# nomadkaraoke/python-audio-separator

Hardware: AMD Instinct MI355X
Metric: audio-sec separated / wall-sec (RTF), UVR-MDX-NET 44.1kHz stereo, 1/2/4/8 GPU (higher is better)
Workload: dtype f32 (I/O and accumulators; matrix products on the 16-bit pipe from block-scaled two-part fp16 operands, 22-bit products -- see arithmetic; fp32-exact setting timed in arithmetic_ab)

## Files before the change

python-audio-separator_amd/csrc/asx.hip:

```cpp
#include <hip/hip_runtime.h>

#include <algorithm>
#include <atomic>
#include <cmath>
#include <cstdarg>
#include <cstdio>
#include <cstdlib>
#include <cstring>
#include <functional>
#include <map>
#include <string>
#include <mutex>
#include <vector>

#include "../../include/asx.h"
#include "knobs.h"

static void grant_lds(const void *kernel, int bytes) {
  static std::mutex mu;
  static std::map<const void *, int> granted;
  std::lock_guard<std::mutex> lock(mu);
  int &g = granted[kernel];
  if (bytes > g) {
    (void)hipFuncSetAttribute(kernel, hipFuncAttributeMaxDynamicSharedMemorySize, bytes);
// ... 27 lines not shown
#include "engine_core.h"
#include "engine_mdx.h"

static int opt_nonneg(int32_t v) { return v < 0 ? 0 : (int)v; }
static int opt_onoff(int32_t v) { return v > 0 ? 1 : 0; }

static const struct EngineOption {
  const char *key;
  int asx_engine::*field;
  int EngineKnobs::*knob;
  int (*norm)(int32_t);
  const char *refusal = nullptr;
  int shipped = 0;
} kOptions[] = {
    {"winograd", &asx_engine::winograd, &EngineKnobs::winograd, opt_nonneg,
     "asx_set_option: winograd = %d names a superseded kernel generation that only an experimental build carries "
     "(python build.py --experimental); this library has 0 (direct kernel) and 3 (the default)", 3},
    {"winograd_stationary", &asx_engine::winos, &EngineKnobs::winos, opt_nonneg,
     "asx_set_option: the weight-stationary Winograd kernel (measured slower) is in experimental builds only (python build.py --experimental)"},
    {"winograd_bf16x6", &asx_engine::wino6, &EngineKnobs::wino6, opt_nonneg},
    {"gemm_bf16x6", &asx_engine::gemm_bf16x6, &EngineKnobs::gemm_bf16x6, opt_onoff},
    {"gemm_f16x3", &asx_engine::gemm_f16x3, &EngineKnobs::gemm_f16x3, opt_onoff},
    {"conv_direct_f16x3", &asx_engine::conv3h, &EngineKnobs::conv3h, opt_nonneg},
    {"conv_down_bf16x6", &asx_engine::down6, &EngineKnobs::down6, opt_onoff},
    {"conv_up_bf16x6", &asx_engine::up6, &EngineKnobs::up6, opt_onoff},
    {"gemm_pair_images", &asx_engine::pair_images, &EngineKnobs::pair_images, opt_onoff,
     "asx_set_option: gemm_pair_images = 1 needs an experimental build (python build.py --experimental): the pair-image reader measured no "
     "faster in the nets and is not in the default library"},
};

static const EngineOption *find_option(const char *fn, const char *key) {
  for (const EngineOption &o : kOptions)
    if (!strcmp(key, o.key)) return &o;
  set_err("%s: unknown option '%s'", fn, key);
  return nullptr;
}

extern "C" {

int asx_abi_version(void) { return ASX_ABI_VERSION; }
const char *asx_last_error(void) { return g_err; }

int asx_device_count(void) {
  int n = 0;
  if (hipGetDeviceCount(&n) != hipSuccess) return 0;
  return n;
// ... 111 lines not shown
    return rc;
  }
  *out = e;
  return ASX_OK;
}

static void v3_destroy(V3Net *n);
static void rof_destroy(RofNet *n);
static void ht_destroy(HtNet *n);
static void hd_destroy(HdNet *n);
static void hd_drop_clones(asx_engine *e);
static void vr_destroy(VrNet *n);
static void ens_destroy(EnsCtx *c);
static void free_conv(ConvLayer &L) {
  L.w.release();
  L.b.release();
  L.wu.release();
  L.wu2.release();
  L.wu3.release();
  L.wus.release();
  L.wu6.release();
  L.wu6h.release();
  L.w3h.release();
  L.wd6.release();
  L.wup6.release();
  L.gn_w.release();
  L.gn_b.release();
}
static void free_tdf(TdfLayer &L) {
  L.w.release();
  L.bias.release();
  L.scale.release();
  L.shift.release();
  L.gn_w.release();
  L.gn_b.release();
}
static void free_block(Block &b) {
  for (auto &c : b.tfc) free_conv(c);
  free_tdf(b.tdf0);
  free_tdf(b.tdf1);
}

void asx_engine_destroy(asx_engine *e) {
  w3_flush(e);
  if (!e) return;
  (void)hipSetDevice(e->device);
// ... 1859 lines not shown
  CHK(vr_plan(*e->vr, n_samples, &T, &n_out));
  DevBuf dw, dp, ds;
  BufGuard g{{&dw, &dp, &ds}};
  CHK(to_dev(dw, wave_host, (size_t)2 * n_samples));
  if (primary_host) CHK(dp.ensure((size_t)2 * n_out * 4));
  if (secondary_host) CHK(ds.ensure((size_t)2 * n_out * 4));
  CHK(vr_separate_dev(e, dw.f(), n_samples, params, primary_host ? dp.f() : nullptr, secondary_host ? ds.f() : nullptr, nullptr));
  if (primary_host) CHK(to_host(primary_host, dp, (size_t)2 * n_out));
  if (secondary_host) CHK(to_host(secondary_host, ds, (size_t)2 * n_out));
  return ASX_OK;
}

int asx_counter(const asx_engine *e, const char *name, int64_t *out) {
  REQUIRE(e && name && out, "asx_counter: null argument");
  const std::string nm(name);
  if (nm == "tdf3_launches") *out = (int64_t)g_tdf3_launches.load();
  else if (nm == "tdf3h_launches") *out = (int64_t)g_tdf3h_launches.load();
  else if (nm == "attn6_launches") *out = (int64_t)g_attn6_launches.load();
  else if (nm == "attn6h_launches") *out = (int64_t)g_attn6h_launches.load();
  else if (nm == "tdf3_gather_launches") *out = (int64_t)g_tdf3_gather_launches.load();
  else if (nm == "wino6_launches") *out = (int64_t)g_wino6_launches.load();
  else if (nm == "wino6h_launches") *out = (int64_t)g_wino6h_launches.load();
  else if (nm == "conv3h_launches") *out = (int64_t)g_conv3h_launches.load();
  else if (nm == "tdf3_pair_image_launches") *out = (int64_t)g_tdf3ps_launches.load();
  else if (nm == "down6_launches") *out = (int64_t)g_down6_launches.load();
  else if (nm == "up6_launches") *out = (int64_t)g_up6_launches.load();
  else if (nm == "hd_rounds") *out = (int64_t)g_hd_rounds.load();
  else {
    set_err("asx_counter: unknown counter '%s'", name);
    return ASX_ERR_INVALID;
  }
  return ASX_OK;
}

int asx_debug_trace(uint64_t *host, int64_t n_u64) {
  REQUIRE(host && n_u64 > 0 && n_u64 <= 4096 * 8, "asx_debug_trace: bad argument");
  HIPCHK(hipDeviceSynchronize());
  HIPCHK(hipMemcpyFromSymbol(host, HIP_SYMBOL(asx_dbg_trace), (size_t)n_u64 * 8));
  return ASX_OK;
}

int asx_debug_fetch(asx_engine *e, const char *name, float *host, int64_t numel) {
  REQUIRE(e && name && host && numel > 0, "asx_debug_fetch: bad argument");
  HIPCHK(hipSetDevice(e->device));
  const float *src = nullptr;
  const std::string nm(name);
// ... 194 lines not shown
```

python-audio-separator_amd/csrc/engine_core.h:

```cpp
#pragma once

static thread_local char g_err[512] = "";
static void set_err(const char *fmt, ...) {
  va_list ap;
  va_start(ap, fmt);
  vsnprintf(g_err, sizeof(g_err), fmt, ap);
  va_end(ap);
}
#define HIPCHK(x)                                                                       \
  do {                                                                                  \
    hipError_t e_ = (x);                                                                \
    if (e_ != hipSuccess) {                                                             \
      set_err("%s:%d %s -> %s", __FILE__, __LINE__, #x, hipGetErrorString(e_));         \
      return ASX_ERR_HIP;                                                               \
    }                                                                                   \
  } while (0)
#define CHK(x)                    \
  do {                            \
    int r_ = (x);                 \
    if (r_ != ASX_OK) return r_;  \
  } while (0)
#define REQUIRE(cond, ...)        \
  do {                            \
    if (!(cond)) {                \
// ... 55 lines not shown
  CHK(run(din.f(), dout.f()));
  return to_host(out_host, dout, n_out);
}

enum ConvKind { CK_3X3 = 0, CK_DOWN = 1, CK_1X1 = 2, CK_UP = 3 };

struct ConvLayer {
  int kind = CK_3X3;
  int cin = 0, cout = 0;
  int nrep = 0, kc = 0, cg = 0, nci = 0;
  int relu = 1;
  DevBuf w, b;
  DevBuf wu;
  DevBuf wu2;
  DevBuf wu3;
  int wu_cg = 0, wu_nci = 0, wu3_nci = 0;
  DevBuf wus;
  int wus_ks = 0;
  DevBuf gn_w, gn_b;
  DevBuf wu6;
  int wu6_nci = 0;
  DevBuf wu6h;
  DevBuf w3h;
  DevBuf wd6;
  int wd6_cg = 0, wd6_nst = 0, wd6_nrep = 3;
  DevBuf wup6;
  int wup6_cg = 0, wup6_nst = 0;
};

struct TdfLayer {
  int n = 0, k = 0, c = 0;
  bool has_bias = false;
  DevBuf w, bias, scale, shift;
  DevBuf gn_w, gn_b;
};

struct Block {
  std::vector<ConvLayer> tfc;
  TdfLayer tdf0, tdf1;
  int c = 0, t = 0, f = 0;
};

struct ProfRec {
  int cls;
  int nprod;
  hipEvent_t a, b;
// ... 49 lines not shown
  bool net_begun = false, net_ready = false;
  asx_net_config net{};
  std::map<std::string, std::vector<float>> host_tensors;
  ConvLayer first, final_;
  std::vector<Block> enc, dec;
  Block mid;
  std::vector<ConvLayer> ds, us;
  int ws_batch = 0;
  DevBuf spec_in, spec_out, R[3], H, HE, frames, chunk_out, d_starts, d_nact, d_peak, d_demixed;
  DevBuf pool_wave, pool_nsong, pool_songs, pool_div, pool_peak;
  DevBuf gn_part;
  DevBuf d_div;
  DivKey div_key;
  DevBuf sinc_tab;
  hipEvent_t div_ev = nullptr;
  hipStream_t div_stream = nullptr;
  std::vector<DevBuf> skip;
  int winograd = 3;
  int winos = 0;
  int gemm_bf16x6 = 1;
  int gemm_f16x3 = 1;
  int wino6 = 144;
  int conv3h = 144;
  int down6 = 1;
  int up6 = 1;
  int pair_images = 0;
  std::vector<W3Entry> w3;
  std::mutex w3_mu;
  bool prof = false;
  int prof_nprod = 0;
  std::vector<ProfRec> recs;
};

static int pick_batch(const asx_engine *e) { return e->cfg.max_batch > 0 ? e->cfg.max_batch : 64; }

static int even_batches(int nk, int maxB) {
  const int nbatch = (nk + maxB - 1) / maxB;
  return (nk + nbatch - 1) / nbatch;
}

template <class F>
static int timed(asx_engine *e, int cls, double flops, double bytes, hipStream_t s, F &&launch) {
  if (!e->prof) {
    launch();
    HIPCHK(hipGetLastError());
    return ASX_OK;
// ... 68 lines not shown
```

python-audio-separator_amd/csrc/engine_mdx.h:

```cpp
#pragma once

template <class CFG>
static void launch_conv_t(const ConvArgs &a, int nblk, hipStream_t s) {
  grant_lds(&conv_mfma_kernel<CFG>, CFG::LDS_BYTES);
  hipLaunchKernelGGL(conv_mfma_kernel<CFG>, dim3(nblk), dim3(256), CFG::LDS_BYTES, s, a);
}

static int conv_tile_h(int kind) { return kind == CK_UP ? 4 : 8; }

static int pick_nrep_conv(int cout) {
  const int ct = (cout + 15) / 16;
  int best = 1, best_pad = 1 << 30;
  for (int n = 3; n >= 1; --n) {
    const int pad = ((ct + n - 1) / n) * n - ct;
    if (pad < best_pad) {
      best_pad = pad;
      best = n;
    }
  }
  return best;
}
static int pick_nrep_up(int cout) {
  const int ct = (cout + 15) / 16;
  if (knobs().up_nrep == 4 && (4 * ct) % 4 == 0) return 4;
// ... 128 lines not shown
#endif
#ifdef ASX_EXPERIMENTAL_KERNELS
    if (L.wus_ks) {
      const size_t per = (size_t)8 * (6 * L.wus_ks / 4) * 64 * 4;
      std::vector<float> wus((size_t)L.wu_cg * per, 0.f);
      for (int co = 0; co < L.cout; ++co)
        for (int c = 0; c < L.cin; ++c) {
          const float *g = &w[((size_t)co * L.cin + c) * 9];
          double t[4][3];
          for (int a = 0; a < 4; ++a)
            for (int j = 0; j < 3; ++j) t[a][j] = G[a][0] * g[0 * 3 + j] + G[a][1] * g[1 * 3 + j] + G[a][2] * g[2 * 3 + j];
          float *dst = &wus[(size_t)(co / 48) * per];
          for (int a = 0; a < 4; ++a)
            for (int bb = 0; bb < 4; ++bb) {
              const float u = (float)(t[a][0] * G[bb][0] + t[a][1] * G[bb][1] + t[a][2] * G[bb][2]);
              dst[L.wus_ks == 12 ? winos_u_index<12>(a, bb, c, co % 48) : winos_u_index<24>(a, bb, c, co % 48)] = u;
            }
        }
      CHK(L.wus.ensure(wus.size() * 4));
      HIPCHK(hipMemcpy(L.wus.p, wus.data(), wus.size() * 4, hipMemcpyHostToDevice));
    }
#endif
  }
  if (L.kind == CK_DOWN) {
    std::vector<uint32_t> w6;
    L.wd6_nrep = (knobs().down6_wide && L.cout % 96 == 0) ? 6 : 3;
    if (L.wd6_nrep == 6) down6_pack<6>(w, L.cout, L.cin, w6, &L.wd6_cg, &L.wd6_nst);
    else down6_pack<3>(w, L.cout, L.cin, w6, &L.wd6_cg, &L.wd6_nst);
    CHK(L.wd6.ensure(w6.size() * 4));
    HIPCHK(hipMemcpy(L.wd6.p, w6.data(), w6.size() * 4, hipMemcpyHostToDevice));
  }
  if (L.kind == CK_UP) {
    std::vector<uint32_t> w6;
    if (L.nrep == 6) up6_pack<6>(w, L.cout, L.cin, w6, &L.wup6_cg, &L.wup6_nst);
    else if (L.nrep == 4) up6_pack<4>(w, L.cout, L.cin, w6, &L.wup6_cg, &L.wup6_nst);
    else up6_pack<2>(w, L.cout, L.cin, w6, &L.wup6_cg, &L.wup6_nst);
    CHK(L.wup6.ensure(w6.size() * 4));
    HIPCHK(hipMemcpy(L.wup6.p, w6.data(), w6.size() * 4, hipMemcpyHostToDevice));
  }
  const int nb = (L.kind == CK_UP) ? CT * 16 : std::max(L.cg * NW, ((L.cout + 47) / 48) * 48);
  std::vector<float> bp(nb, 0.f);
  for (int i = 0; i < L.cout; ++i) bp[i] = b ? b[i] : 0.f;
  CHK(L.w.ensure(wp.size() * 4));
  CHK(L.b.ensure(bp.size() * 4));
  HIPCHK(hipMemcpy(L.w.p, wp.data(), wp.size() * 4, hipMemcpyHostToDevice));
  HIPCHK(hipMemcpy(L.b.p, bp.data(), bp.size() * 4, hipMemcpyHostToDevice));
  return ASX_OK;
}

template <class CFG>
static void launch_conv_dma_t(const ConvArgs &a, int nblk, hipStream_t s) {
  grant_lds(&conv_dma_kernel<CFG>, CFG::LDS_BYTES);
  hipLaunchKernelGGL(conv_dma_kernel<CFG>, dim3(nblk), dim3(256), CFG::LDS_BYTES, s, a);
}

static std::atomic<long long> g_wino6_launches{0};
static std::atomic<long long> g_wino6h_launches{0};
static std::atomic<long long> g_conv3h_launches{0};
static std::atomic<long long> g_down6_launches{0};
static std::atomic<long long> g_up6_launches{0};

struct ConvView {
  int64_t x_bstride = 0;
  int64_t y_bstride = 0;
  const float *res = nullptr;
  int64_t aux_bstride = 0;
  int act = -1;
  float alpha = 1.f;
};

static int conv_launch(asx_engine *e, const ConvLayer &L, const float *x, const float *skip, float *y, int B, int T,
                       int F, hipStream_t s, const ConvView &v = ConvView()) {
  ConvArgs a{};
  a.x = x;
  a.wp = L.w.f();
  a.bias = L.b.f();
  a.skip = skip;
  a.res = v.res;
  a.zeros = e->d_zeros.f();
  a.y = y;
  a.B = B;
  a.Cin = L.cin;
  a.Cout = L.cout;
  a.T = T;
  a.F = F;
  a.act = v.act >= 0 ? v.act : (L.relu ? ACT_RELU : ACT_NONE);
  a.alpha = v.alpha;
  REQUIRE(a.act != ACT_ELU || L.kind == CK_1X1, "ELU epilogue: 1x1 convolutions only");
  a.CG = L.cg;
  a.NCI = L.nci;
  a.nt = knobs().nt & 1;
  int cls = ASX_PROF_CONV3X3;
// ... 12 lines not shown
    if (L.kind == CK_1X1) {
      cls = ASX_PROF_CONV1X1;
      taps = 1;
    } else if (L.kind == CK_UP) {
      cls = ASX_PROF_UP;
      taps = 4;
      out_plane = (int64_t)4 * T * F;
    }
  }
  a.x_bstride = v.x_bstride ? v.x_bstride : (int64_t)L.cin * T * F;
  a.y_bstride = v.y_bstride ? v.y_bstride : (int64_t)L.cout * out_plane;
  a.aux_bstride = v.aux_bstride ? v.aux_bstride : (int64_t)L.cout * out_plane;
  const int th = conv_tile_h(L.kind);
  a.tilesT = (a.To + th - 1) / th;
  a.tilesF = (a.Fo + 63) / 64;
  const int nblk = a.CG * a.tilesT * a.tilesF * B;
  if (nblk <= 0) return ASX_OK;
  const double outpix = (double)B * a.To * a.Fo;
  const double flops = 2.0 * taps * L.cin * L.cout * outpix;
  double bytes = 4.0 * ((double)B * L.cin * T * F + (double)L.cout * outpix * (L.kind == CK_UP ? 4 : 1));
  if (L.kind == CK_UP && skip) bytes += 4.0 * (double)L.cout * outpix * 4;
  if (v.res) bytes += 4.0 * (double)L.cout * outpix;
  int bad = 0;
  const bool dma = (F % 4 == 0) && ((reinterpret_cast<uintptr_t>(x) & 15) == 0) && (a.x_bstride % 4 == 0) && !knobs().no_dma;
  const ConvArgs &d = a;
#ifdef ASX_EXPERIMENTAL_KERNELS
  if (L.kind == CK_3X3 && e->winograd == 3 && e->winos == 1 && dma && L.wus.p != nullptr && a.Fo % 32 == 0 && v.res == nullptr &&
      (a.act == ACT_RELU || a.act == ACT_NONE) && (int64_t)L.cin * T * F < ((int64_t)1 << 30)) {
    ConvArgs wa = a;
    wa.wp = L.wus.f();
    wa.CG = L.wu_cg;
    wa.tilesF = a.Fo / 32;
    const int NS = (a.To + 1) / 2;
    const int base = wa.CG * wa.tilesF * B;
    int RB = std::max(1, std::min((NS + 7) / 8, (2048 + base - 1) / base));
    const int SPB = (NS + RB - 1) / RB;
    RB = (NS + SPB - 1) / SPB;
    wa.tilesT = RB;
    wa.NCI = SPB;
    const int nb = base * RB;
    auto gos = [&](auto kern, int lds) {
      grant_lds(kern, lds);
      return timed(e, cls, flops, bytes, s, [&]() { hipLaunchKernelGGL(kern, dim3(nb), dim3(512), lds, s, wa); });
    };
    const int abls = knobs().winos_abl;
    const bool k12 = L.wus_ks == 12;
    const bool ragged = (a.To & 1) || (L.cout % 48) != 0;
    if (abls && !ragged) {
      switch (abls) {
        case 1: return k12 ? gos(&conv_winos_kernel<12, 1>, WinoSCfg<12>::LDS_BYTES) : gos(&conv_winos_kernel<24, 1>, WinoSCfg<24>::LDS_BYTES);
        case 2: return k12 ? gos(&conv_winos_kernel<12, 2>, WinoSCfg<12>::LDS_BYTES) : gos(&conv_winos_kernel<24, 2>, WinoSCfg<24>::LDS_BYTES);
        case 4: return k12 ? gos(&conv_winos_kernel<12, 4>, WinoSCfg<12>::LDS_BYTES) : gos(&conv_winos_kernel<24, 4>, WinoSCfg<24>::LDS_BYTES);
        case 5: return k12 ? gos(&conv_winos_kernel<12, 5>, WinoSCfg<12>::LDS_BYTES) : gos(&conv_winos_kernel<24, 5>, WinoSCfg<24>::LDS_BYTES);
        case 13: return k12 ? gos(&conv_winos_kernel<12, 13>, WinoSCfg<12>::LDS_BYTES) : gos(&conv_winos_kernel<24, 13>, WinoSCfg<24>::LDS_BYTES);
        default: break;
      }
    }
    if (ragged) return k12 ? gos(&conv_winos_kernel<12, 0, true>, WinoSCfg<12>::LDS_BYTES) : gos(&conv_winos_kernel<24, 0, true>, WinoSCfg<24>::LDS_BYTES);
    return k12 ? gos(&conv_winos_kernel<12, 0, false>, WinoSCfg<12>::LDS_BYTES) : gos(&conv_winos_kernel<24, 0, false>, WinoSCfg<24>::LDS_BYTES);
  }
#endif
  if (L.kind == CK_3X3 && e->winograd == 3 && e->gemm_bf16x6 > 0 && e->gemm_f16x3 > 0 && e->conv3h > 0 && L.cin <= e->conv3h && L.w3h.p != nullptr && dma &&
      v.res == nullptr && (a.act == ACT_RELU || a.act == ACT_NONE) && F % 32 == 0 && (int64_t)Conv3hCfg::C * T * F < ((int64_t)1 << 29) &&
      a.y_bstride % 4 == 0 && (reinterpret_cast<uintptr_t>(y) & 15) == 0) {
    const int nb = L.cin / Conv3hCfg::C;
    const int tilesT = (T + 3) / 4, tilesF = F / 32;
    int bw = 32;
    double best = 1e30;
    for (int cand : {32, 16, 8}) {
      if ((tilesT * cand) % 32 != 0) continue;
      const int tps = tilesT * cand / 32;
      const int bands = (tilesF + cand - 1) / cand, items = B * bands;
      const double cost = (double)(bands * cand) / tilesF * (tps + 1.0) / tps * (double)((items + 7) / 8) / (items / 8.0);
      if (cost < best - 1e-9) {
        best = cost;
        bw = cand;
      }
    }
    if (best > 1e29) bw = 32;
    grant_lds(&conv3h_kernel<0, false>, Conv3hCfg::LDS_BYTES);
    grant_lds(&conv3h_kernel<0, true>, Conv3hCfg::LDS_BYTES);
    const int64_t plane = (int64_t)T * F;
    return timed(e, cls, flops, bytes, s, [&]() {
      e->prof_nprod = 3;
      for (int ob = 0; ob < nb; ++ob)
        for (int ib = 0; ib < nb; ++ib) {
          Conv3hArgs ca{};
          ca.x = x + (int64_t)ib * Conv3hCfg::C * plane;
          ca.y = y + (int64_t)ob * Conv3hCfg::C * plane;
          ca.prev = ib > 0 ? ca.y : nullptr;
          ca.wimg = reinterpret_cast<const u32x4 *>(reinterpret_cast<const uint32_t *>(L.w3h.p) + (size_t)(ob * nb + ib) * Conv3hCfg::IMG_U32);
          ca.bias = ib == 0 ? L.b.f() + ob * Conv3hCfg::C : nullptr;
          ca.B = B;
          ca.T = T;
          ca.F = F;
          ca.x_bstride = a.x_bstride;
          ca.y_bstride = a.y_bstride;
          ca.act = ib == nb - 1 ? a.act : ACT_NONE;
          ca.tilesT = tilesT;
          ca.tilesF = tilesF;
          ca.bw = bw;
          ca.tps = (tilesT * bw) % 32 == 0 ? tilesT * bw / 32 : tilesT;
          if (ib > 0) hipLaunchKernelGGL((conv3h_kernel<0, true>), dim3(256), dim3(512), Conv3hCfg::LDS_BYTES, s, ca);
          else hipLaunchKernelGGL((conv3h_kernel<0, false>), dim3(256), dim3(512), Conv3hCfg::LDS_BYTES, s, ca);
          g_conv3h_launches.fetch_add(1);
        }
    });
  }
  if (L.kind == CK_3X3 && e->winograd == 3 && e->gemm_bf16x6 > 0 && e->wino6 > 0 && L.cin >= e->wino6 && dma && L.wu6_nci > 0 &&
      (int64_t)T * F < ((int64_t)1 << 24)) {
    ConvArgs wa = a;
    const bool h3 = e->gemm_f16x3 > 0 && L.wu6h.p != nullptr;
    wa.wp = reinterpret_cast<const float *>(h3 ? L.wu6h.p : L.wu6.p);
    wa.CG = L.wu_cg;
    wa.NCI = L.wu6_nci;
    wa.tilesT = (a.To + Wino6Cfg::TH - 1) / Wino6Cfg::TH;
    wa.tilesF = (a.Fo + Wino6Cfg::TW - 1) / Wino6Cfg::TW;
    const int64_t S = (int64_t)wa.tilesT * wa.tilesF * B;
    const int64_t nb = ((S + 7) / 8) * 8 * wa.CG;
    if (nb < ((int64_t)1 << 31)) {
      grant_lds(&conv_wino6_kernel<0, 1>, Wino6Cfg::LDS_BYTES);
      grant_lds(&conv_wino6_kernel<0, 1, true>, Wino6Cfg::LDS_BYTES);
      g_wino6_launches.fetch_add(1);
      if (h3) g_wino6h_launches.fetch_add(1);
      return timed(e, cls, flops, bytes, s, [&]() {
        e->prof_nprod = h3 ? 3 : 6;
// ... 655 lines not shown
      else hipLaunchKernelGGL(f3::istft3p_kernel<0>, dim3(ng, 2, B), dim3(256), f3::ISTFT3P_LDS_BYTES, s, f);
    }
    else
      hipLaunchKernelGGL(f3::istft3_kernel, dim3(ng, 2, B), dim3(256), f3::ISTFT3_LDS_BYTES, s, f);
    if (ng > 1) hipLaunchKernelGGL(f3::seam3_kernel, dim3(5, ng - 1, B * 2), dim3(256), 0, s, f);
  });
}

static int gn_launch(asx_engine *e, const float *x, int B, int C, int64_t P, const DevBuf &gw, const DevBuf &gb, const float *res,
                     const float *mul, float *y, hipStream_t s) {
  if (B <= 0) return ASX_OK;
  REQUIRE(C % 2 == 0 && gw.p && gb.p && e->gn_part.bytes >= (size_t)B * C * 16, "GroupNorm(2, %d): channels / workspace", C);
  double2 *part = reinterpret_cast<double2 *>(e->gn_part.p);
  const double bytes = 4.0 * (double)B * C * (double)P;
  CHK(timed(e, ASX_PROF_MISC, 0.0, bytes, s,
            [&]() { hipLaunchKernelGGL(gn_partial_kernel, dim3((unsigned)C, (unsigned)B), dim3(256), 0, s, x, C, P, part); }));
  const int nx = (int)std::max<int64_t>(1, std::min<int64_t>(32, (P / 4 + 1023) / 1024));
  return timed(e, ASX_PROF_MISC, 0.0, bytes * (2 + (res ? 1 : 0) + (mul ? 1 : 0)), s, [&]() {
    hipLaunchKernelGGL(gn_apply_kernel, dim3((unsigned)nx, (unsigned)C, (unsigned)B), dim3(256), 0, s, x, C, 2, P, part, gw.f(), gb.f(), 1e-5f, 1, res,
                       mul, y);
  });
}

static int block_forward(asx_engine *e, const Block &blk, float *&cur, float *dest, int B, hipStream_t s) {
  auto next_free = [&](const float *a, const float *b) -> float * {
    for (int i = 0; i < 3; ++i)
      if (e->R[i].f() != a && e->R[i].f() != b) return e->R[i].f();
    return nullptr;
  };
  const bool gn = e->net.norm == 1;
  const int64_t plane = (int64_t)blk.t * blk.f;
  for (size_t j = 0; j < blk.tfc.size(); ++j) {
    float *out = next_free(cur, nullptr);
    CHK(conv_launch(e, blk.tfc[j], cur, nullptr, out, B, blk.t, blk.f, s));
    if (gn) CHK(gn_launch(e, out, B, blk.c, plane, blk.tfc[j].gn_w, blk.tfc[j].gn_b, nullptr, nullptr, out, s));
    cur = out;
  }
  const int64_t M = (int64_t)B * blk.c * blk.t;
  const int bnk = e->net.bn;
  if (bnk < 0) {
    if (dest) {
      HIPCHK(hipMemcpyAsync(dest, cur, (size_t)M * blk.f * 4, hipMemcpyDeviceToDevice, s));
      cur = dest;
    }
    return ASX_OK;
  }
  if (bnk == 0) {
    float *out = dest ? dest : next_free(cur, nullptr);
    if (gn) {
      float *tmp = next_free(cur, out);
      CHK(tdf_launch(e, blk.tdf0, cur, nullptr, tmp, M, blk.t, s, 0));
      CHK(gn_launch(e, tmp, B, blk.c, plane, blk.tdf0.gn_w, blk.tdf0.gn_b, cur, nullptr, out, s));
    } else {
      CHK(tdf_launch(e, blk.tdf0, cur, cur, out, M, blk.t, s));
    }
    cur = out;
    return ASX_OK;
// ... 3 lines not shown
    CHK(gn_launch(e, e->H.f(), B, blk.c, (int64_t)blk.t * (blk.f / bnk), blk.tdf0.gn_w, blk.tdf0.gn_b, nullptr, nullptr, e->H.f(), s));
    float *out = dest ? dest : next_free(cur, nullptr);
    float *tmp = dest ? next_free(cur, nullptr) : out;
    CHK(tdf_launch(e, blk.tdf1, e->H.f(), nullptr, tmp, M, blk.t, s, 0));
    CHK(gn_launch(e, tmp, B, blk.c, plane, blk.tdf1.gn_w, blk.tdf1.gn_b, cur, nullptr, out, s));
    cur = out;
    return ASX_OK;
  }
  float *out = dest ? dest : (knobs().tdf_inplace ? cur : next_free(cur, nullptr));
  CHK(tdf_pair_launch(e, blk.tdf0, blk.tdf1, cur, e->H.f(), reinterpret_cast<int *>(e->HE.p), out, M, blk.t, s));
  cur = out;
  return ASX_OK;
}

static int net_forward_dev(asx_engine *e, const float *spec_in, float *spec_out, int B, hipStream_t s) {
  if (!e->net_ready) {
    set_err("net weights not committed");
    return ASX_ERR_STATE;
  }
  const int T = e->net.dim_t, F = e->net.dim_f;
  const int n = e->net.num_blocks / 2;
  const bool gn = e->net.norm == 1;
  float *cur = e->R[0].f();
  CHK(conv_launch(e, e->first, spec_in, nullptr, cur, B, T, F, s));
  if (gn) CHK(gn_launch(e, cur, B, e->net.g, (int64_t)T * F, e->first.gn_w, e->first.gn_b, nullptr, nullptr, cur, s));
  for (int i = 0; i < n; ++i) {
    CHK(block_forward(e, e->enc[i], cur, e->skip[i].f(), B, s));
    float *out = e->R[0].f();
    CHK(conv_launch(e, e->ds[i], cur, nullptr, out, B, e->enc[i].t, e->enc[i].f, s));
    if (gn)
      CHK(gn_launch(e, out, B, e->ds[i].cout, (int64_t)(e->enc[i].t / 2) * (e->enc[i].f / 2), e->ds[i].gn_w, e->ds[i].gn_b, nullptr, nullptr, out, s));
    cur = out;
  }
  CHK(block_forward(e, e->mid, cur, nullptr, B, s));
  for (int i = 0; i < n; ++i) {
    const Block &blk = e->dec[i];
    float *out = nullptr;
    for (int r = 0; r < 3; ++r)
      if (e->R[r].f() != cur) {
        out = e->R[r].f();
        break;
      }
    CHK(conv_launch(e, e->us[i], cur, gn ? nullptr : e->skip[n - 1 - i].f(), out, B, blk.t / 2, blk.f / 2, s));
    if (gn)
      CHK(gn_launch(e, out, B, e->us[i].cout, (int64_t)blk.t * blk.f, e->us[i].gn_w, e->us[i].gn_b, nullptr, e->skip[n - 1 - i].f(), out, s));
    cur = out;
    CHK(block_forward(e, blk, cur, nullptr, B, s));
  }
  CHK(conv_launch(e, e->final_, cur, nullptr, spec_out, B, T, F, s));
  return ASX_OK;
}

static int ensure_workspace(asx_engine *e, int Bchunks, bool need_net) {
  const int T = e->cfg.segment_size, Fq = e->cfg.dim_f;
  const int mult = (need_net && e->cfg.enable_denoise) ? 2 : 1;
  const size_t Bn = (size_t)Bchunks * mult;
  CHK(e->spec_in.ensure(Bn * 4 * T * Fq * 4));
// ... 20 lines not shown
```

python-audio-separator_amd/csrc/kernels_conv3h.h:

```cpp
#pragma once
#include <cstring>
#include <vector>

#include "kernels_gemm3.h"

namespace asx {

struct Conv3hArgs {
  const float *x;
  float *y;
  const u32x4 *wimg;
  const float *bias;
  int B, T, F;
  int64_t x_bstride, y_bstride;
  int act;
  int tilesT, tilesF;
  int bw, tps;
  const float *prev;
  long long *dbg;
};

struct Conv3hCfg {
  static constexpr int C = 48, CG8 = C / 8;
  static constexpr int TH = 4, TW = 32, IW = TW + 2;
  static constexpr int PSTR = C * 2;
  static constexpr int ROWB = IW * PSTR;
  static constexpr int RING = 12;
  static constexpr int PART = RING * ROWB;
  static constexpr int KGY = 3 * CG8;
  static constexpr int SPK = (KGY + 3) / 4;
  static constexpr int NST = 3 * SPK;
  static constexpr int WKY = (KGY / 4) * 3 * 2 * 1024 + 3 * 2 * 512;
  static constexpr int WBYTES = 3 * WKY;
  static constexpr int W_OFF = 0, X_OFF = WBYTES, TAB_OFF = X_OFF + 2 * PART;
  static constexpr int LDS_BYTES = TAB_OFF + 64;
  static constexpr size_t IMG_U32 = WBYTES / 4 + 48;
  static constexpr int EUP = 8;
};

inline uint16_t conv3h_f16_rne(float f) {
  uint32_t x;
  memcpy(&x, &f, 4);
// ... 114 lines not shown
__device__ __forceinline__ void conv3h_walk_next(const Conv3hArgs &a, int wg, Conv3hWalk &w) {
  if (++w.j == a.tps) {
    w.j = -1;
    w.item += 8;
    conv3h_walk_item(a, wg, w);
  }
}

__device__ __forceinline__ void conv3h_split_pair(float x0, float x1, float s, unsigned &h, unsigned &l) {
  unsigned hh = 0, ll = 0;
  asm("v_fma_mixlo_f16 %0, %1, %2, 0 op_sel_hi:[0,0,0]" : "+v"(hh) : "v"(x0), "v"(s));
  asm("v_fma_mixhi_f16 %0, %1, %2, 0 op_sel_hi:[0,0,0]" : "+v"(hh) : "v"(x1), "v"(s));
  asm("v_fma_mixlo_f16 %0, %1, %2, -%3 op_sel:[0,0,0] op_sel_hi:[0,0,1]" : "+v"(ll) : "v"(x0), "v"(s), "v"(hh));
  asm("v_fma_mixhi_f16 %0, %1, %2, -%3 op_sel:[0,0,1] op_sel_hi:[0,0,1]" : "+v"(ll) : "v"(x1), "v"(s), "v"(hh));
  h = hh;
  l = ll;
}

template <int BM>
__device__ __forceinline__ float ror8m(float keep, float from) {
  return __builtin_bit_cast(float, __builtin_amdgcn_update_dpp(__builtin_bit_cast(int, keep), __builtin_bit_cast(int, from), 0x128, 0xf, BM, false));
}

template <int ABL = 0, bool ACC = false>
__global__ __launch_bounds__(512) __attribute__((amdgpu_waves_per_eu(2, 2))) void conv3h_kernel(Conv3hArgs a) {
  using CFG = Conv3hCfg;
  extern __shared__ float lds_f[];
  char *lds = reinterpret_cast<char *>(lds_f);
  const int tid = threadIdx.x;
  const int lane = tid & 63;
  const int wave = __builtin_amdgcn_readfirstlane(tid >> 6);
  const int wg = blockIdx.x;
  float *maxtab = reinterpret_cast<float *>(lds + CFG::TAB_OFF);
  int *exps = reinterpret_cast<int *>(lds + CFG::TAB_OFF + 32);

  {
    const u32x4 *src = a.wimg;
    u32x4 *dst = reinterpret_cast<u32x4 *>(lds + CFG::W_OFF);
    for (int i = tid; i < CFG::WBYTES / 16; i += 512) dst[i] = src[i];
  }
  const int64_t TF = (int64_t)a.T * a.F;
  const int NB = conv3h_nblocks(a, wg);
  const int row0 = conv3h_row0(a, wg);
  const unsigned plane_bytes = (unsigned)(CFG::C * TF * 4);

  if (wave >= 4) {
    const int ptid = tid - 256, pw = wave - 4;
    int row, cig, q;
    if (ptid < 160) {
      q = (ptid & 1) + 2 * ((ptid >> 3) % 5);
      cig = (ptid >> 1) & 3;
      row = ptid / 40;
    } else {
      const int u = ptid - 160;
      q = (u & 1) + 2 * ((u >> 3) % 5);
      cig = 4 + ((u >> 1) & 1);
      row = ((u >> 2) & 1) + 2 * (u / 40);
    }
    const bool item_ok = ptid < 240;
    const int loff = (row * CFG::IW + 4 * q - 3) * CFG::PSTR + cig * 16;
    const int goff = (int)(((int64_t)cig * 8 * a.T + row) * a.F + 4 * q);
    f32x4 raw[4][8];

    Conv3hWalk wk;
    conv3h_walk_init(a, wg, wk);
    int nf = 0;
    auto fetch = [&](auto setc) {
      constexpr int S = decltype(setc)::value;
      const int tb = nf < NB ? wk.b : 0, f0 = wk.strip * 32;
      const int t1 = nf < NB ? row0 + wk.j * 4 + 1 : -(1 << 20);
      ++nf;
      conv3h_walk_next(a, wg, wk);
      __amdgpu_buffer_rsrc_t rs = __builtin_amdgcn_make_buffer_rsrc(const_cast<float *>(a.x + (int64_t)tb * a.x_bstride), 0, plane_bytes, 0x00020000);
      const int org = t1 * a.F + (f0 - 4);
      const bool ok = item_ok && (unsigned)(t1 + row) < (unsigned)a.T && (unsigned)(f0 - 4 + 4 * q) < (unsigned)a.F;
      const unsigned vo = ok ? (unsigned)(goff + org) * 4u : 0xfffffff0u;
#pragma unroll
      for (int j = 0; j < 8; ++j) {
        if constexpr ((ABL & 2) != 0) raw[S][j] = (f32x4){0.25f, 0.5f, 0.75f, 1.f};
        else raw[S][j] = __builtin_bit_cast(f32x4, __builtin_amdgcn_raw_buffer_load_b128(rs, (int)vo, (int)(j * TF * 4), 0));
      }
    };
    auto tile_max = [&](auto setc, int slot) {
      constexpr int S = decltype(setc)::value;
      float m = 0.f;
#pragma unroll
      for (int j = 0; j < 8; ++j) {
        m = __builtin_fmaxf(__builtin_fmaxf(m, __builtin_fabsf(raw[S][j].x)), __builtin_fabsf(raw[S][j].y));
        m = __builtin_fmaxf(__builtin_fmaxf(m, __builtin_fabsf(raw[S][j].z)), __builtin_fabsf(raw[S][j].w));
      }
      m = wave_max64(m);
      if (!(m <= 3.4028234663852886e38f)) {
        m = 0.f;
#pragma unroll
        for (int j = 0; j < 8; ++j) {
          m = fmaxf(m, fmaxf(fmaxf(finite_or_zero(raw[S][j].x), finite_or_zero(raw[S][j].y)), fmaxf(finite_or_zero(raw[S][j].z), finite_or_zero(raw[S][j].w))));
        }
        m = wave_max64(m);
      }
      if (lane == 0) maxtab[slot * 4 + pw] = m;
    };
    int e_prev = 0, js = -1;
    auto split_store = [&](auto setc, int par, int slot3) {
      constexpr int S = decltype(setc)::value;
      const f32x4 mv = *reinterpret_cast<const f32x4 *>(maxtab + par * 4);
      const float m = fmaxf(fmaxf(mv.x, mv.y), fmaxf(mv.z, mv.w));
      int need = f16_scale_exp(m) - 1;
      need = need < 100 ? need : 100;
      int e = e_prev;
      if (js < 0 || need < e_prev) e = need;
      else if (need > e_prev + CFG::EUP) e = need < e_prev + 40 ? need : e_prev + 40;
      e_prev = e;
      if (++js == a.tps) js = -1;
      if (ptid == 0) exps[slot3] = e;
      const float sc = __builtin_ldexpf(1.0f, e);
      char *dst = lds + CFG::X_OFF + slot3 * 4 * CFG::ROWB + loff;
      if constexpr ((ABL & 8) != 0) return;
#pragma unroll
      for (int i = 0; i < 4; ++i) {
        unsigned hh[4], ll[4];
#pragma unroll
        for (int c2 = 0; c2 < 4; ++c2) conv3h_split_pair(raw[S][2 * c2][i], raw[S][2 * c2 + 1][i], sc, hh[c2], ll[c2]);
        const bool wok = item_ok && (i == 3 ? q <= 8 : (i == 0 ? q >= 1 : (q >= 1 && q <= 8)));
        if (wok) {
          *reinterpret_cast<u32x4 *>(dst + i * CFG::PSTR) = (u32x4){hh[0], hh[1], hh[2], hh[3]};
          *reinterpret_cast<u32x4 *>(dst + CFG::PART + i * CFG::PSTR) = (u32x4){ll[0], ll[1], ll[2], ll[3]};
        }
// ... 286 lines not shown
```

python-audio-separator_amd/csrc/knobs.h:

```cpp
#pragma once

#include <algorithm>
#include <climits>
#include <cstdint>
#include <cstdlib>

#ifndef ASX_TDF2_DEFAULT
#define ASX_TDF2_DEFAULT 1
#endif

constexpr int HD_MAX_GROUPS = 6;

namespace knob {
inline bool set(const char *name) { return getenv(name) != nullptr; }
inline int num(const char *name, int def) { return set(name) ? atoi(getenv(name)) : def; }
inline int64_t num64(const char *name, int64_t def) { return set(name) ? atoll(getenv(name)) : def; }
inline double real(const char *name, double def) { return set(name) ? atof(getenv(name)) : def; }
inline bool on_unless_0(const char *name) { return !(set(name) && atoi(getenv(name)) == 0); }
inline bool off_unless_nonzero(const char *name) { return set(name) && atoi(getenv(name)) != 0; }
inline int clamped(const char *name, int def, int lo, int hi = INT_MAX) { return set(name) ? std::max(lo, std::min(hi, atoi(getenv(name)))) : def; }
}

struct Knobs {
  int poison = knob::num("ASX_POISON", -1);
// ... 57 lines not shown
  int rof_gelu = knob::num("ASX_ROF_GELU", 2);
  bool rof_fuse = knob::on_unless_0("ASX_ROF_FUSE");
};

inline const Knobs &knobs() {
  static const Knobs k;
  return k;
}

struct EngineKnobs {
#ifdef ASX_EXPERIMENTAL_KERNELS
  int winograd = knob::clamped("ASX_WINOGRAD", 3, 0);
  int winos = knob::clamped("ASX_WINOS", 0, 0);
  int pair_images = knob::num("ASX_PAIR_IMAGES", 0);
#else
  int winograd = knob::num("ASX_WINOGRAD", 3) <= 0 ? 0 : 3;
  int winos = 0;
  int pair_images = 0;
#endif
  int gemm_bf16x6 = knob::num("ASX_GEMM_BF16X6", 1);
  int gemm_f16x3 = knob::num("ASX_GEMM_F16X3", 1);
  int wino6 = knob::clamped("ASX_WINO6", 144, 0);
  int conv3h = knob::clamped("ASX_CONV3H", 144, 0);
  int down6 = knob::num("ASX_DOWN6", 1);
  int up6 = knob::num("ASX_UP6", 1);
  bool fft3 = knob::on_unless_0("ASX_FFT3");
  bool fft3p = knob::on_unless_0("ASX_FFT3P");
};
```

Before: 1556.

## Fuse first 1x1 input conv into the following conv3h 3x3 kernel

```diff
diff --git a/python-audio-separator_amd/csrc/asx.hip b/python-audio-separator_amd/csrc/asx.hip
--- a/python-audio-separator_amd/csrc/asx.hip
+++ b/python-audio-separator_amd/csrc/asx.hip
@@ -73,6 +73,7 @@
     {"gemm_bf16x6", &asx_engine::gemm_bf16x6, &EngineKnobs::gemm_bf16x6, opt_onoff},
     {"gemm_f16x3", &asx_engine::gemm_f16x3, &EngineKnobs::gemm_f16x3, opt_onoff},
     {"conv_direct_f16x3", &asx_engine::conv3h, &EngineKnobs::conv3h, opt_nonneg},
+    {"conv_fuse_input", &asx_engine::conv_fuse_input, &EngineKnobs::conv_fuse_input, opt_onoff},
     {"conv_down_bf16x6", &asx_engine::down6, &EngineKnobs::down6, opt_onoff},
     {"conv_up_bf16x6", &asx_engine::up6, &EngineKnobs::up6, opt_onoff},
     {"gemm_pair_images", &asx_engine::pair_images, &EngineKnobs::pair_images, opt_onoff,
@@ -230,6 +231,7 @@
   L.wu6.release();
   L.wu6h.release();
   L.w3h.release();
+  L.w1f.release();
   L.wd6.release();
   L.wup6.release();
   L.gn_w.release();
@@ -2135,6 +2137,7 @@
   else if (nm == "wino6_launches") *out = (int64_t)g_wino6_launches.load();
   else if (nm == "wino6h_launches") *out = (int64_t)g_wino6h_launches.load();
   else if (nm == "conv3h_launches") *out = (int64_t)g_conv3h_launches.load();
+  else if (nm == "conv3h_fin_launches") *out = (int64_t)g_conv3h_fin_launches.load();
   else if (nm == "tdf3_pair_image_launches") *out = (int64_t)g_tdf3ps_launches.load();
   else if (nm == "down6_launches") *out = (int64_t)g_down6_launches.load();
   else if (nm == "up6_launches") *out = (int64_t)g_up6_launches.load();
diff --git a/python-audio-separator_amd/csrc/engine_core.h b/python-audio-separator_amd/csrc/engine_core.h
--- a/python-audio-separator_amd/csrc/engine_core.h
+++ b/python-audio-separator_amd/csrc/engine_core.h
@@ -101,6 +101,7 @@
   int wu6_nci = 0;
   DevBuf wu6h;
   DevBuf w3h;
+  DevBuf w1f;
   DevBuf wd6;
   int wd6_cg = 0, wd6_nst = 0, wd6_nrep = 3;
   DevBuf wup6;
@@ -196,6 +197,7 @@
   int gemm_f16x3 = 1;
   int wino6 = 144;
   int conv3h = 144;
+  int conv_fuse_input = 1;
   int down6 = 1;
   int up6 = 1;
   int pair_images = 0;
diff --git a/python-audio-separator_amd/csrc/engine_mdx.h b/python-audio-separator_amd/csrc/engine_mdx.h
--- a/python-audio-separator_amd/csrc/engine_mdx.h
+++ b/python-audio-separator_amd/csrc/engine_mdx.h
@@ -174,6 +174,13 @@
     }
 #endif
   }
+  if (L.kind == CK_1X1 && L.cin == 4 && L.cout == Conv3hCfg::C) {
+    std::vector<float> w1((size_t)Conv3hCfg::C * 5, 0.f);
+    memcpy(w1.data(), w, (size_t)Conv3hCfg::C * 4 * 4);
+    if (b) memcpy(w1.data() + Conv3hCfg::C * 4, b, (size_t)Conv3hCfg::C * 4);
+    CHK(L.w1f.ensure(w1.size() * 4));
+    HIPCHK(hipMemcpy(L.w1f.p, w1.data(), w1.size() * 4, hipMemcpyHostToDevice));
+  }
   if (L.kind == CK_DOWN) {
     std::vector<uint32_t> w6;
     L.wd6_nrep = (knobs().down6_wide && L.cout % 96 == 0) ? 6 : 3;
@@ -209,6 +216,7 @@
 static std::atomic<long long> g_wino6_launches{0};
 static std::atomic<long long> g_wino6h_launches{0};
 static std::atomic<long long> g_conv3h_launches{0};
+static std::atomic<long long> g_conv3h_fin_launches{0};
 static std::atomic<long long> g_down6_launches{0};
 static std::atomic<long long> g_up6_launches{0};
 
@@ -219,7 +227,18 @@
   int64_t aux_bstride = 0;
   int act = -1;
   float alpha = 1.f;
+  const ConvLayer *fin = nullptr;
+  const float *fin_x = nullptr;
 };
+
+static bool conv3h_takes(const asx_engine *e, const ConvLayer &L, bool dma, const float *res, int act, int T, int F, int64_t y_bstride, const float *y) {
+#ifdef ASX_EXPERIMENTAL_KERNELS
+  if (e->winos == 1 && L.wus.p != nullptr) return false;
+#endif
+  return L.kind == CK_3X3 && e->winograd == 3 && e->gemm_bf16x6 > 0 && e->gemm_f16x3 > 0 && e->conv3h > 0 && L.cin <= e->conv3h && L.w3h.p != nullptr && dma &&
+         res == nullptr && (act == ACT_RELU || act == ACT_NONE) && F % 32 == 0 && (int64_t)Conv3hCfg::C * T * F < ((int64_t)1 << 29) &&
+         y_bstride % 4 == 0 && (reinterpret_cast<uintptr_t>(y) & 15) == 0;
+}
 
 static int conv_launch(asx_engine *e, const ConvLayer &L, const float *x, const float *skip, float *y, int B, int T,
                        int F, hipStream_t s, const ConvView &v = ConvView()) {
@@ -278,7 +297,9 @@
   if (L.kind == CK_UP && skip) bytes += 4.0 * (double)L.cout * outpix * 4;
   if (v.res) bytes += 4.0 * (double)L.cout * outpix;
   int bad = 0;
-  const bool dma = (F % 4 == 0) && ((reinterpret_cast<uintptr_t>(x) & 15) == 0) && (a.x_bstride % 4 == 0) && !knobs().no_dma;
+  const bool dma = (F % 4 == 0) && ((reinterpret_cast<uintptr_t>(v.fin ? v.fin_x : x) & 15) == 0) && (a.x_bstride % 4 == 0) && !knobs().no_dma;
+  REQUIRE(!v.fin || (v.fin->w1f.p != nullptr && L.cin == Conv3hCfg::C && conv3h_takes(e, L, dma, v.res, a.act, T, F, a.y_bstride, y)),
+          "fused-input 3x3 conv: the layer does not run conv3h_kernel");
   const ConvArgs &d = a;
 #ifdef ASX_EXPERIMENTAL_KERNELS
   if (L.kind == CK_3X3 && e->winograd == 3 && e->winos == 1 && dma && L.wus.p != nullptr && a.Fo % 32 == 0 && v.res == nullptr &&
@@ -316,9 +337,7 @@
     return k12 ? gos(&conv_winos_kernel<12, 0, false>, WinoSCfg<12>::LDS_BYTES) : gos(&conv_winos_kernel<24, 0, false>, WinoSCfg<24>::LDS_BYTES);
   }
 #endif
-  if (L.kind == CK_3X3 && e->winograd == 3 && e->gemm_bf16x6 > 0 && e->gemm_f16x3 > 0 && e->conv3h > 0 && L.cin <= e->conv3h && L.w3h.p != nullptr && dma &&
-      v.res == nullptr && (a.act == ACT_RELU || a.act == ACT_NONE) && F % 32 == 0 && (int64_t)Conv3hCfg::C * T * F < ((int64_t)1 << 29) &&
-      a.y_bstride % 4 == 0 && (reinterpret_cast<uintptr_t>(y) & 15) == 0) {
+  if (conv3h_takes(e, L, dma, v.res, a.act, T, F, a.y_bstride, y)) {
     const int nb = L.cin / Conv3hCfg::C;
     const int tilesT = (T + 3) / 4, tilesF = F / 32;
     int bw = 32;
@@ -336,6 +355,7 @@
     if (best > 1e29) bw = 32;
     grant_lds(&conv3h_kernel<0, false>, Conv3hCfg::LDS_BYTES);
     grant_lds(&conv3h_kernel<0, true>, Conv3hCfg::LDS_BYTES);
+    grant_lds(&conv3h_kernel<0, false, true>, Conv3hCfg::LDS_BYTES);
     const int64_t plane = (int64_t)T * F;
     return timed(e, cls, flops, bytes, s, [&]() {
       e->prof_nprod = 3;
@@ -357,7 +377,13 @@
           ca.tilesF = tilesF;
           ca.bw = bw;
           ca.tps = (tilesT * bw) % 32 == 0 ? tilesT * bw / 32 : tilesT;
-          if (ib > 0) hipLaunchKernelGGL((conv3h_kernel<0, true>), dim3(256), dim3(512), Conv3hCfg::LDS_BYTES, s, ca);
+          if (v.fin) {
+            ca.xin = v.fin_x;
+            ca.xin_bstride = 4 * plane;
+            ca.w1 = v.fin->w1f.f();
+            hipLaunchKernelGGL((conv3h_kernel<0, false, true>), dim3(256), dim3(512), Conv3hCfg::LDS_BYTES, s, ca);
+            g_conv3h_fin_launches.fetch_add(1);
+          } else if (ib > 0) hipLaunchKernelGGL((conv3h_kernel<0, true>), dim3(256), dim3(512), Conv3hCfg::LDS_BYTES, s, ca);
           else hipLaunchKernelGGL((conv3h_kernel<0, false>), dim3(256), dim3(512), Conv3hCfg::LDS_BYTES, s, ca);
           g_conv3h_launches.fetch_add(1);
         }
@@ -1059,7 +1085,7 @@
   });
 }
 
-static int block_forward(asx_engine *e, const Block &blk, float *&cur, float *dest, int B, hipStream_t s) {
+static int block_forward(asx_engine *e, const Block &blk, float *&cur, float *dest, int B, hipStream_t s, const float *fin_x = nullptr) {
   auto next_free = [&](const float *a, const float *b) -> float * {
     for (int i = 0; i < 3; ++i)
       if (e->R[i].f() != a && e->R[i].f() != b) return e->R[i].f();
@@ -1069,7 +1095,12 @@
   const int64_t plane = (int64_t)blk.t * blk.f;
   for (size_t j = 0; j < blk.tfc.size(); ++j) {
     float *out = next_free(cur, nullptr);
-    CHK(conv_launch(e, blk.tfc[j], cur, nullptr, out, B, blk.t, blk.f, s));
+    ConvView v;
+    if (j == 0 && fin_x) {
+      v.fin = &e->first;
+      v.fin_x = fin_x;
+    }
+    CHK(conv_launch(e, blk.tfc[j], cur, nullptr, out, B, blk.t, blk.f, s, v));
     if (gn) CHK(gn_launch(e, out, B, blk.c, plane, blk.tfc[j].gn_w, blk.tfc[j].gn_b, nullptr, nullptr, out, s));
     cur = out;
   }
@@ -1119,17 +1150,25 @@
   const int n = e->net.num_blocks / 2;
   const bool gn = e->net.norm == 1;
   float *cur = e->R[0].f();
-  CHK(conv_launch(e, e->first, spec_in, nullptr, cur, B, T, F, s));
-  if (gn) CHK(gn_launch(e, cur, B, e->net.g, (int64_t)T * F, e->first.gn_w, e->first.gn_b, nullptr, nullptr, cur, s));
+  const Block &blk0 = n > 0 ? e->enc[0] : e->mid;
+  const bool fuse = e->conv_fuse_input > 0 && !gn && e->first.kind == CK_1X1 && e->first.cin == 4 && e->first.cout == Conv3hCfg::C && e->first.relu &&
+                    e->first.w1f.p != nullptr && !blk0.tfc.empty() && blk0.tfc[0].cin == Conv3hCfg::C && blk0.tfc[0].cout == Conv3hCfg::C &&
+                    conv3h_takes(e, blk0.tfc[0], F % 4 == 0 && (reinterpret_cast<uintptr_t>(spec_in) & 15) == 0 && !knobs().no_dma, nullptr,
+                                 blk0.tfc[0].relu ? ACT_RELU : ACT_NONE, T, F, (int64_t)Conv3hCfg::C * T * F, e->R[1].f());
+  if (!fuse) {
+    CHK(conv_launch(e, e->first, spec_in, nullptr, cur, B, T, F, s));
+    if (gn) CHK(gn_launch(e, cur, B, e->net.g, (int64_t)T * F, e->first.gn_w, e->first.gn_b, nullptr, nullptr, cur, s));
+  }
+  const float *fin_x = fuse ? spec_in : nullptr;
   for (int i = 0; i < n; ++i) {
-    CHK(block_forward(e, e->enc[i], cur, e->skip[i].f(), B, s));
+    CHK(block_forward(e, e->enc[i], cur, e->skip[i].f(), B, s, i == 0 ? fin_x : nullptr));
     float *out = e->R[0].f();
     CHK(conv_launch(e, e->ds[i], cur, nullptr, out, B, e->enc[i].t, e->enc[i].f, s));
     if (gn)
       CHK(gn_launch(e, out, B, e->ds[i].cout, (int64_t)(e->enc[i].t / 2) * (e->enc[i].f / 2), e->ds[i].gn_w, e->ds[i].gn_b, nullptr, nullptr, out, s));
     cur = out;
   }
-  CHK(block_forward(e, e->mid, cur, nullptr, B, s));
+  CHK(block_forward(e, e->mid, cur, nullptr, B, s, n == 0 ? fin_x : nullptr));
   for (int i = 0; i < n; ++i) {
     const Block &blk = e->dec[i];
     float *out = nullptr;
diff --git a/python-audio-separator_amd/csrc/kernels_conv3h.h b/python-audio-separator_amd/csrc/kernels_conv3h.h
--- a/python-audio-separator_amd/csrc/kernels_conv3h.h
+++ b/python-audio-separator_amd/csrc/kernels_conv3h.h
@@ -18,6 +18,9 @@
   int bw, tps;
   const float *prev;
   long long *dbg;
+  const float *xin;
+  const float *w1;
+  int64_t xin_bstride;
 };
 
 struct Conv3hCfg {
@@ -178,7 +181,16 @@
   return __builtin_bit_cast(float, __builtin_amdgcn_update_dpp(__builtin_bit_cast(int, keep), __builtin_bit_cast(int, from), 0x128, 0xf, BM, false));
 }
 
-template <int ABL = 0, bool ACC = false>
+template <bool FIN>
+struct Conv3hFinRegs {};
+template <>
+struct Conv3hFinRegs<true> {
+  f32x4 rin[4][4];
+  bool ok[4];
+  float w1[8][4], b1[8];
+};
+
+template <int ABL = 0, bool ACC = false, bool FIN = false>
 __global__ __launch_bounds__(512) __attribute__((amdgpu_waves_per_eu(2, 2))) void conv3h_kernel(Conv3hArgs a) {
   using CFG = Conv3hCfg;
   extern __shared__ float lds_f[];
@@ -215,8 +227,23 @@
     }
     const bool item_ok = ptid < 240;
     const int loff = (row * CFG::IW + 4 * q - 3) * CFG::PSTR + cig * 16;
-    const int goff = (int)(((int64_t)cig * 8 * a.T + row) * a.F + 4 * q);
-    f32x4 raw[4][8];
+    const int goff = FIN ? (int)((int64_t)row * a.F + 4 * q)
+                         : (int)(((int64_t)cig * 8 * a.T + row) * a.F + 4 * q);
+    constexpr int NSET = FIN ? 2 : 4;
+    f32x4 raw[NSET][8];
+    Conv3hFinRegs<FIN> fr;
+    const unsigned in_bytes = (unsigned)(4 * TF * 4);
+    if constexpr (FIN) {
+#pragma unroll
+      for (int c = 0; c < 8; ++c) {
+        const f32x4 wv = *reinterpret_cast<const f32x4 *>(a.w1 + (cig * 8 + c) * 4);
+        fr.w1[c][0] = wv.x;
+        fr.w1[c][1] = wv.y;
+        fr.w1[c][2] = wv.z;
+        fr.w1[c][3] = wv.w;
+        fr.b1[c] = a.w1[CFG::C * 4 + cig * 8 + c];
+      }
+    }
 
     Conv3hWalk wk;
     conv3h_walk_init(a, wg, wk);
@@ -227,18 +254,36 @@
       const int t1 = nf < NB ? row0 + wk.j * 4 + 1 : -(1 << 20);
       ++nf;
       conv3h_walk_next(a, wg, wk);
-      __amdgpu_buffer_rsrc_t rs = __builtin_amdgcn_make_buffer_rsrc(const_cast<float *>(a.x + (int64_t)tb * a.x_bstride), 0, plane_bytes, 0x00020000);
+      __amdgpu_buffer_rsrc_t rs = FIN ? __builtin_amdgcn_make_buffer_rsrc(const_cast<float *>(a.xin + (int64_t)tb * a.xin_bstride), 0, in_bytes, 0x00020000)
+                                      : __builtin_amdgcn_make_buffer_rsrc(const_cast<float *>(a.x + (int64_t)tb * a.x_bstride), 0, plane_bytes, 0x00020000);
       const int org = t1 * a.F + (f0 - 4);
       const bool ok = item_ok && (unsigned)(t1 + row) < (unsigned)a.T && (unsigned)(f0 - 4 + 4 * q) < (unsigned)a.F;
       const unsigned vo = ok ? (unsigned)(goff + org) * 4u : 0xfffffff0u;
-#pragma unroll
-      for (int j = 0; j < 8; ++j) {
-        if constexpr ((ABL & 2) != 0) raw[S][j] = (f32x4){0.25f, 0.5f, 0.75f, 1.f};
-        else raw[S][j] = __builtin_bit_cast(f32x4, __builtin_amdgcn_raw_buffer_load_b128(rs, (int)vo, (int)(j * TF * 4), 0));
+      if constexpr (FIN) {
+        fr.ok[S] = ok;
+#pragma unroll
+        for (int j = 0; j < 4; ++j) fr.rin[S][j] = __builtin_bit_cast(f32x4, __builtin_amdgcn_raw_buffer_load_b128(rs, (int)vo, (int)(j * TF * 4), 0));
+      } else {
+#pragma unroll
+        for (int j = 0; j < 8; ++j) {
+          if constexpr ((ABL & 2) != 0) raw[S][j] = (f32x4){0.25f, 0.5f, 0.75f, 1.f};
+          else raw[S][j] = __builtin_bit_cast(f32x4, __builtin_amdgcn_raw_buffer_load_b128(rs, (int)vo, (int)(j * TF * 4), 0));
+        }
       }
     };
     auto tile_max = [&](auto setc, int slot) {
-      constexpr int S = decltype(setc)::value;
+      constexpr int S = decltype(setc)::value % NSET;
+      if constexpr (FIN) {
+        constexpr int SI = decltype(setc)::value;
+        const bool ok = fr.ok[SI];
+        auto px = [&](float i0, float i1, float i2, float i3, int c) {
+          const float v = __builtin_fmaf(fr.w1[c][3], i3, __builtin_fmaf(fr.w1[c][2], i2, __builtin_fmaf(fr.w1[c][1], i1, __builtin_fmaf(fr.w1[c][0], i0, fr.b1[c]))));
+          return ok ? __builtin_fmaxf(v, 0.f) : 0.f;
+        };
+        const f32x4 i0 = fr.rin[SI][0], i1 = fr.rin[SI][1], i2 = fr.rin[SI][2], i3 = fr.rin[SI][3];
+#pragma unroll
+        for (int c = 0; c < 8; ++c) raw[S][c] = (f32x4){px(i0.x, i1.x, i2.x, i3.x, c), px(i0.y, i1.y, i2.y, i3.y, c), px(i0.z, i1.z, i2.z, i3.z, c), px(i0.w, i1.w, i2.w, i3.w, c)};
+      }
       float m = 0.f;
 #pragma unroll
       for (int j = 0; j < 8; ++j) {
@@ -258,7 +303,7 @@
     };
     int e_prev = 0, js = -1;
     auto split_store = [&](auto setc, int par, int slot3) {
-      constexpr int S = decltype(setc)::value;
+      constexpr int S = decltype(setc)::value % NSET;
       const f32x4 mv = *reinterpret_cast<const f32x4 *>(maxtab + par * 4);
       const float m = fmaxf(fmaxf(mv.x, mv.y), fmaxf(mv.z, mv.w));
       int need = f16_scale_exp(m) - 1;
diff --git a/python-audio-separator_amd/csrc/knobs.h b/python-audio-separator_amd/csrc/knobs.h
--- a/python-audio-separator_amd/csrc/knobs.h
+++ b/python-audio-separator_amd/csrc/knobs.h
@@ -103,6 +103,7 @@
   int gemm_f16x3 = knob::num("ASX_GEMM_F16X3", 1);
   int wino6 = knob::clamped("ASX_WINO6", 144, 0);
   int conv3h = knob::clamped("ASX_CONV3H", 144, 0);
+  int conv_fuse_input = 1;
   int down6 = knob::num("ASX_DOWN6", 1);
   int up6 = knob::num("ASX_UP6", 1);
   bool fft3 = knob::on_unless_0("ASX_FFT3");
```

Measured after the change: 1579, median of 6. 1.02x the previous value.
